# raymondclowe/EasyWakeWord

Hardware: NVIDIA B200
Metric: audio-sec/sec MFCC+cosine-match @4096 streams, 1/2/4/8 B200; % HBM peak (higher is better)
Workload: dtype f32

## Files before the change

easywakeword_b200/_lib.py:

```python
from __future__ import annotations

import ctypes as C
import os

import numpy as np

HERE = os.path.dirname(os.path.abspath(__file__))
LIB_PATH = os.path.join(HERE, "libewk.so")

EWK_OK, EWK_ERR_ARG, EWK_ERR_NO_TEMPLATE, EWK_ERR_CUDA, EWK_ERR_STATE, EWK_ERR_NOMEM = 0, -1, -2, -3, -4, -5
PCM_F32, PCM_I16 = 0, 1
IN_ULAW, IN_ALAW = 2, 3
HOST, DEVICE = 0, 1


class EwkError(RuntimeError):
    pass


class Config(C.Structure):
    _fields_ = [("n_streams", C.c_int32), ("ring_samples", C.c_int32), ("slack_samples", C.c_int32),
                ("pcm_format", C.c_int32), ("max_templates", C.c_int32), ("max_events", C.c_int32),
                ("preemphasis", C.c_float), ("n_mfcc", C.c_int32), ("reserved0", C.c_int32), ("reserved1", C.c_int32)]

# ... 267 lines not shown
        "ewk_push_g711": (C.c_int, [vp, i32, i32, vp, i64, i64, i32, i32]),
        "ewk_push_resampled": (C.c_int, [vp, i32, i32, vp, i32, i64, i64, i32, i32]),
        "ewk_push_resampled_each": (C.c_int, [vp, i32, i32, vp, i32, i64, i64, i32, i32, _p(i64)]),
        "ewk_push_streams": (C.c_int, [vp, _p(C.c_int32), i32, vp, i32, _p(i64), _p(i64), i64, i32, i32, _p(i64)]),
        "ewk_tick_ready": (C.c_int, [vp, i32, _p(C.c_int32), vp, vp, vp, vp]),
        "ewk_stream_input": (C.c_int, [vp, i32, _p(C.c_int32), _p(i64)]),
        "ewk_reset_streams": (C.c_int, [vp, _p(C.c_int32), i32]),
        "ewk_tick": (C.c_int, [vp, i32]),
        "ewk_set_overlap": (C.c_int, [vp, i32]),
        "ewk_join": (C.c_int, [vp]),
        "ewk_tick_trace": (C.c_int, [vp, i32, vp, vp, vp, vp]),
        "ewk_poll": (C.c_int, [vp, vp, i32, _p(C.c_int)]),
        "ewk_stream_status_get": (C.c_int, [vp, i32, _p(StreamStatus)]),
        "ewk_read_last": (C.c_int, [vp, i32, i64, f32p]),
        "ewk_read_segment": (C.c_int, [vp, i32, i64, i64, f32p]),
        "ewk_stream_results": (C.c_int, [vp, vp]),
        "ewk_dense_scores": (C.c_int, [vp, i64, i32, i32, i32, vp, i32]),
        "ewk_dense_scores_streams": (C.c_int, [vp, _p(C.c_int32), i32, _p(i64), _p(C.c_int32), i32, i32, vp, i64, i32]),
        "ewk_dense_ready": (C.c_int, [vp, _p(C.c_int32), i32, i32, i32, i32, _p(i64), _p(C.c_int32), vp, i64, i32]),
        "ewk_dense_detect": (C.c_int, [vp, _p(C.c_int32), i32, i32, i32, i32, i32, i32, vp, i32, _p(i64), _p(C.c_int32),
                                       vp, i64, i32]),
        "ewk_prepare_segments": (C.c_int, [vp, i32, _p(C.c_int32), _p(i64), _p(i64), _p(i64), f32p, i64, i32]),
        "ewk_results_device_ptr": (C.c_int, [vp, _p(vp)]),
        "ewk_set_results_buffer": (C.c_int, [vp, vp]),
        "ewk_set_results_peers": (C.c_int, [vp, _p(vp), i32, i64, i64, _p(vp), i32]),
        "ewk_publish_parity": (C.c_int, [vp]),
        "ewk_publish_seq": (C.c_int64, [vp]),
        "ewk_wait_published": (C.c_int, [vp, i32, i64, i32]),
        "ewk_published_seq": (C.c_int, [vp, i32, _p(C.c_uint64), i32]),
        "ewk_match_stream": (C.c_int, [vp, _p(vp)]),
        "ewk_host_alloc": (C.c_int, [_p(vp), i64]),
        "ewk_host_free": (C.c_int, [vp]),
        "ewk_launch_count": (C.c_int64, [vp]),
        "ewk_profile": (C.c_int, [vp, i32]),
        "ewk_profile_read": (C.c_int, [vp, _p(C.c_double), _p(C.c_int64)]),
    }
    for name, (res, args) in protos.items():
        fn = getattr(lib, name)
        fn.restype = res
        fn.argtypes = args
    lib._protos.update(protos)


_orig_load = load


def load():
    lib = _orig_load()
    if "ewk_push" not in lib._protos:
        _declare_stream_protos(lib)
    return lib


def default_stream_params(**over):
    lib = load()
    p = StreamParams()
    lib.ewk_default_stream_params(C.byref(p))
    for k, v in over.items():
        if not hasattr(p, k):
            raise TypeError(f"unknown stream parameter {k!r}")
        setattr(p, k, v)
    return p


class PinnedArray:

# ... 330 lines not shown
            signals = list(signals)
            if len(signals) != len(bases):
                raise ValueError("one signal row per destination")
            sig = (C.c_void_p * max(1, len(signals)))(*[C.c_void_p(int(b)) for b in signals])
        self._ck(self.lib.ewk_set_results_peers(self.h, arr, len(bases), int(stride_records), int(offset_records), sig, int(slot)))

    def publish_parity(self):
        return int(self.lib.ewk_publish_parity(self.h))

    def publish_seq(self):
        return int(self.lib.ewk_publish_seq(self.h))

    def wait_published(self, n_slots, seq, timeout_ms=2000):
        self._ck(self.lib.ewk_wait_published(self.h, int(n_slots), int(seq), int(timeout_ms)))

    def published_seq(self, parity, n_slots):
        out = np.zeros(n_slots, np.uint64)
        rc = self.lib.ewk_published_seq(self.h, int(parity), out.ctypes.data_as(_p(C.c_uint64)), int(n_slots))
        if rc < 0:
            self._ck(rc)
        return out, bool(rc)

    def match_stream(self):
        p = C.c_void_p()
        self._ck(self.lib.ewk_match_stream(self.h, C.byref(p)))
        return p.value or 0

    def set_cuda_stream(self, handle):
        self._ck(self.lib.ewk_set_cuda_stream(self.h, C.c_void_p(handle)))

    def launch_count(self):
        return int(self.lib.ewk_launch_count(self.h))

    def profile(self, enable=True):
        self._ck(self.lib.ewk_profile(self.h, 1 if enable else 0))

    def profile_read(self):
        ms = (C.c_double * 8)()
        n = (C.c_int64 * 8)()
        self._ck(self.lib.ewk_profile_read(self.h, ms, n))
        names = ["ring_push", "tick_gate", "segment_queue", "segment_batch", "dense_score", "segment_prepare", "publish",
                 "resample_push"]
        return {names[i]: {"ms": ms[i], "launches": int(n[i])} for i in range(len(names))}

    for f in (prepare_segments, dense_scores, dense_scores_streams, dense_ready, dense_detect, dense_last_plan, profile, profile_read, set_stream_params, push, push_g711, push_resampled,
              push_resampled_each, push_streams, tick_ready, reset_streams, stream_input, tick, poll, status, read_last, read_segment, results, results_device_ptr,
              set_results_buffer, set_results_peers, publish_parity, publish_seq, wait_published, published_seq, match_stream, set_cuda_stream, launch_count):
        setattr(Context, f.__name__, f)


_bank_methods()
```

easywakeword_b200/csrc/ewk_api.cu:

```cuda
#include <cuda_runtime.h>

#include <algorithm>
#include <cmath>
#include <climits>
#include <cstdarg>
#include <cstdio>
#include <cstdlib>
#include <cstring>
#include <string>
#include <type_traits>
#include <vector>

#include "../../include/ewk.h"
#include "ewk_ctx.hpp"

using namespace ewk;

static thread_local std::string g_create_error = "";

void ewk_ctx::fail(const char* fmt, ...) {
    char buf[1024];
    va_list ap;
    va_start(ap, fmt);
    vsnprintf(buf, sizeof(buf), fmt, ap);
// ... 516 lines not shown
    p->frame_size = 0;
    p->pre_speech_silence = 0.8;
    p->speech_duration_min = 0.3;
    p->speech_duration_max = 2.0;
    p->post_speech_silence = 0.4;
    p->timeout = 30.0;
    p->min_threshold = 0.005;
    p->template_first = 0;
    p->template_count = 1;
    p->live = 0;
    return EWK_OK;
}

int ewk_ctx::init_streams() {
    ewk_ctx* ctx = this;
    const int n = cfg.n_streams;
    if (n == 0) return EWK_OK;
    const size_t esz = cfg.pcm_format == EWK_PCM_I16 ? 2 : 4;
    bank.n_streams = n;
    bank.R = cfg.ring_samples;
    bank.P = ((cfg.ring_samples + cfg.slack_samples + 63) / 64) * 64;
    bank.fmt = cfg.pcm_format == EWK_PCM_I16 ? 1 : 0;
    chunk_cap = std::max(1, cfg.ring_samples / MIN_FRAME_SIZE);
    bank.chunk_cap = chunk_cap;
    bank.max_events = std::max(16, cfg.max_events);
    CK(cudaMalloc(&bank.ring, esz * (size_t)n * bank.P));
    CK(cudaMemsetAsync(bank.ring, 0, esz * (size_t)n * bank.P, stream));
    CK(cudaMalloc(&bank.st, sizeof(StreamState) * (size_t)n));
    CK(cudaMalloc(&bank.prm, sizeof(StreamParams) * (size_t)n));
    CK(cudaMalloc(&bank.chunk_ms, sizeof(double) * (size_t)n * 2 * chunk_cap));
    CK(cudaMalloc(&bank.events, sizeof(EventRec) * (size_t)bank.max_events));
    CK(cudaMalloc(&bank.ev_count, sizeof(int) * 8));
    CK(cudaMemsetAsync(bank.ev_count, 0, sizeof(int) * 8, stream));
    CK(cudaMalloc(&bank.bk_count, sizeof(int) * SEG_NB));
    CK(cudaMemsetAsync(bank.bk_count, 0, sizeof(int) * SEG_NB, stream));
    CK(cudaMalloc(&bank.bk_list, sizeof(int) * (size_t)SEG_NB * bank.max_events));
#ifdef EWK_K3_TRACE
    if (getenv("EWK_K3_TRACE")) {
        CK(cudaMalloc(&bank.k3_trace, sizeof(long long) * K3_TRACE_WORDS * (size_t)queue_grid()));
        CK(cudaMemsetAsync(bank.k3_trace, 0, sizeof(long long) * K3_TRACE_WORDS * (size_t)queue_grid(), stream));
    }
#endif

    bank.NB = bank.P / TICK;
    CK(cudaMalloc(&bank.block_ss, sizeof(double) * (size_t)n * std::max(1, bank.NB)));
    CK(cudaMalloc(&own_results, sizeof(StreamResult) * (size_t)n));
    bank.results = (StreamResult*)own_results;
    if (const char* e = getenv("EWK_K3")) k3_frames = atoi(e) == 2;
    if (!k3_frames) {
        if (use_lm) CK(cudaMalloc(&bank.lm_ws, sizeof(float) * (size_t)queue_grid() * SEG_SMEM_FRAMES * LM_ROW));
    } else {
        const size_t cap = std::min<size_t>((size_t)bank.max_events * SEG_SMEM_FRAMES, ((size_t)2 << 30) / (FROW * sizeof(float)));
        bank.frow_cap = (int)cap;
        CK(cudaMalloc(&bank.frow, sizeof(float) * FROW * cap));
        CK(cudaMalloc(&bank.frame_ev, sizeof(int) * cap));
        CK(cudaMalloc(&bank.ev_done, sizeof(int) * (size_t)bank.max_events));
    }
    std::vector<StreamState> st(n);
    std::memset(st.data(), 0, sizeof(StreamState) * n);
    for (auto& x : st) { x.thr = 0.01; x.last_ev = -1; }
    CK(cudaMemcpyAsync(bank.st, st.data(), sizeof(StreamState) * n, cudaMemcpyHostToDevice, stream));
    ewk_stream_params dp;
    ewk_default_stream_params(&dp);
    StreamParams sp;
    std::memcpy(&sp, &dp, sizeof(sp));
    h_prm.assign(n, sp);
    max_post = sp.post_speech_silence;
    CK(cudaMemcpyAsync(bank.prm, h_prm.data(), sizeof(StreamParams) * n, cudaMemcpyHostToDevice, stream));
    std::vector<StreamResult> rs(n);
    for (auto& r : rs) { r.score = std::nanf(""); r.flags = 0; }
    CK(cudaMemcpyAsync(bank.results, rs.data(), sizeof(StreamResult) * n, cudaMemcpyHostToDevice, stream));
    CK(cudaStreamSynchronize(stream));
    h_written.assign(n, 0);
    h_visible_lb.assign(n, 0);
    h_tick.assign(n, 0);
    h_dense_next.assign(n, 1);
    h_det_next.assign(n, 1);
    h_frame_size.assign(n, 0);
    h_rate.assign(n, 0);
    h_inputs.assign(n, 0);
    CK(cudaFuncSetAttribute(segment_queue_kernel<false>, cudaFuncAttributeMaxDynamicSharedMemorySize,
                            (int)seg_smem_bytes(SEG_SMEM_FRAMES)));
    CK(cudaFuncSetAttribute(segment_queue_kernel<true>, cudaFuncAttributeMaxDynamicSharedMemorySize,
                            (int)seg_smem_bytes(SEG_SMEM_FRAMES)));
    CK(cudaFuncSetAttribute(segment_frames_kernel<false>, cudaFuncAttributeMaxDynamicSharedMemorySize, (int)fq_smem_bytes()));
    CK(cudaFuncSetAttribute(segment_frames_kernel<true>, cudaFuncAttributeMaxDynamicSharedMemorySize, (int)fq_smem_bytes()));
    CK(cudaFuncSetAttribute(ring_push_bulk_kernel<short>, cudaFuncAttributeMaxDynamicSharedMemorySize, 112 * 1024));
    CK(cudaFuncSetAttribute(ring_push_bulk_kernel<float>, cudaFuncAttributeMaxDynamicSharedMemorySize, 112 * 1024));
    {
        const size_t big = sizeof(double) * 3 * (size_t)(std::min(chunk_cap, GATE_SMEM_CHUNKS) + 1) * GATE_WARPS;
        const size_t staged = sizeof(double) * 3 * (size_t)130 * GATE_WARPS + (size_t)2 * TICK * 4 * GATE_WARPS;
        CK(cudaFuncSetAttribute(tick_gate_kernel<false>, cudaFuncAttributeMaxDynamicSharedMemorySize, (int)std::max(big, staged)));
        CK(cudaFuncSetAttribute(tick_gate_kernel<true>, cudaFuncAttributeMaxDynamicSharedMemorySize, (int)std::max(big, staged)));
    }
    return EWK_OK;
}

void ewk_ctx::release_streams() {
#ifdef EWK_K3_TRACE
    if (bank.k3_trace) {
        cudaDeviceSynchronize();
        std::vector<long long> h((size_t)K3_TRACE_WORDS * queue_grid());
        cudaMemcpy(h.data(), bank.k3_trace, h.size() * sizeof(long long), cudaMemcpyDeviceToHost);
        if (FILE* f = fopen(getenv("EWK_K3_TRACE"), "wb")) { fwrite(h.data(), sizeof(long long), h.size(), f); fclose(f); }
        cudaFree(bank.k3_trace);
    }
#endif
    if (d_rs_tail) { cudaFree(d_rs_tail); d_rs_tail = nullptr; rs_tail_cap = 0; }
    for (void* p : {bank.ring, (void*)bank.st, (void*)bank.prm, (void*)bank.chunk_ms, (void*)bank.events,
                    (void*)bank.ev_count, (void*)bank.block_ss, (void*)bank.lm_ws, own_results, (void*)bank.frow,
                    (void*)bank.frame_ev, (void*)bank.ev_done, (void*)bank.bk_count, (void*)bank.bk_list})
        if (p) cudaFree(p);
    bank = BankView{};
    own_results = nullptr;
    b_trace.free(); b_read.free(); b_dense.free(); b_keep_rows.free(); b_keep_end.free(); b_g2.free(); b_det_state.free();
    for (auto& p : prof_pairs) { cudaEventDestroy(p.a); cudaEventDestroy(p.b); }
    for (auto e : prof_free) cudaEventDestroy(e);
    prof_pairs.clear(); prof_free.clear();
}

int ewk_ctx::gate_chunks() const {
    int m = 1;
    for (int s = 0; s < bank.n_streams; s++) {
        const int fs = h_frame_size[s] > 0 ? h_frame_size[s] : h_prm[s].frame_size;
        if (fs > 0) m = std::max(m, std::min(bank.chunk_cap, bank.R / fs));
    }
    return m;
}

int ewk_ctx::join_match() {
    ewk_ctx* ctx = this;
    if (!match_inflight) return EWK_OK;
    match_inflight = false;
    CK(cudaStreamWaitEvent(stream, ev_match, 0));
    return EWK_OK;
}

static int need_streams(ewk_ctx* ctx, const char* who, bool join = true) {
    if (ctx->bank.n_streams == 0) { ctx->fail("%s: context was created with n_streams = 0", who); return EWK_ERR_STATE; }
    if (join) return ctx->join_match();
    return EWK_OK;
}

extern "C" int ewk_set_overlap(ewk_ctx* ctx, int enable) {
    if (!ctx) return EWK_ERR_ARG;
    int rc = need_streams(ctx, "ewk_set_overlap");
    if (rc) return rc;
    CK(cudaSetDevice(ctx->device));
    if (enable && !ctx->match_stream) {
        CK(cudaStreamCreateWithFlags(&ctx->match_stream, cudaStreamNonBlocking));
        CK(cudaEventCreateWithFlags(&ctx->ev_gate, cudaEventDisableTiming));
        CK(cudaEventCreateWithFlags(&ctx->ev_match, cudaEventDisableTiming));
    }
    ctx->overlap = enable != 0;
    return EWK_OK;
}

extern "C" int ewk_join(ewk_ctx* ctx) {
    if (!ctx) return EWK_ERR_ARG;
    CK(cudaSetDevice(ctx->device));
    return ctx->join_match();
}

extern "C" int64_t ewk_launch_count(const ewk_ctx* ctx) { return ctx ? ctx->launches : 0; }

extern "C" int ewk_set_stream_params(ewk_ctx* ctx, int stream, const ewk_stream_params* p) {
    if (!ctx) return EWK_ERR_ARG;
    int rc = need_streams(ctx, "ewk_set_stream_params");
    if (rc) return rc;
    const int n = ctx->bank.n_streams;
    if (!p || stream < -1 || stream >= n) { ctx->fail("ewk_set_stream_params: bad stream %d", stream); return EWK_ERR_ARG; }
    if (!(p->pre_speech_silence > 0)) { ctx->fail("pre_speech_silence must be positive"); return EWK_ERR_ARG; }
    if (!(p->speech_duration_min > 0)) { ctx->fail("speech_duration_min must be positive"); return EWK_ERR_ARG; }
    if (!(p->speech_duration_max > 0)) { ctx->fail("speech_duration_max must be positive"); return EWK_ERR_ARG; }
    if (p->speech_duration_min > p->speech_duration_max) { ctx->fail("speech_duration_min must be <= speech_duration_max"); return EWK_ERR_ARG; }
    if (!(p->post_speech_silence > 0)) { ctx->fail("post_speech_silence must be positive"); return EWK_ERR_ARG; }
    if (p->frame_size != 0 && (p->frame_size < MIN_FRAME_SIZE || p->frame_size > ctx->bank.R)) {
        ctx->fail("frame_size must be 0 or in [%d, %d]", MIN_FRAME_SIZE, ctx->bank.R);
        return EWK_ERR_ARG;
    }
    if (p->template_first < 0 || p->template_count < 0 || p->template_first + p->template_count > ctx->cfg.max_templates) {
        ctx->fail("template range [%d, %d) outside [0, %d)", p->template_first, p->template_first + p->template_count, ctx->cfg.max_templates);
        return EWK_ERR_ARG;
    }
    CK(cudaSetDevice(ctx->device));
    StreamParams sp;
    std::memcpy(&sp, p, sizeof(sp));
    const int a = stream < 0 ? 0 : stream, b = stream < 0 ? n : stream + 1;
    for (int s = a; s < b; s++) ctx->h_prm[s] = sp;
    ctx->max_post = 0.0;
    for (int s = 0; s < n; s++) ctx->max_post = std::max(ctx->max_post, ctx->h_prm[s].post_speech_silence);
    CK(cudaMemcpyAsync(ctx->bank.prm + a, ctx->h_prm.data() + a, sizeof(StreamParams) * (size_t)(b - a),
                       cudaMemcpyHostToDevice, ctx->stream));
    CK(cudaStreamSynchronize(ctx->stream));
    return EWK_OK;
}

// ... 675 lines not shown
    const bool want = silent || state || thr || rms;
    const size_t cells = (size_t)B.n_streams * n_ticks;
    if (want) {
        CK(ctx->b_trace.ensure(cells * (2 + 16)));
        char* base = (char*)ctx->b_trace.p;
        tr.thr = (double*)base;
        tr.rms = (double*)(base + cells * 8);
        tr.silent = (unsigned char*)(base + cells * 16);
        tr.state = (unsigned char*)(base + cells * 17);
        if (paced) CK(cudaMemsetAsync(ctx->b_trace.p, 0xFF, cells * (2 + 16), ctx->stream));
    }
    int smem_chunks = ctx->gate_chunks();
    if (smem_chunks > GATE_SMEM_CHUNKS) {
        ctx->fail("ewk_tick: ring_samples / frame_size = %d chunks; the gate keeps them in shared memory and supports at most %d "
                  "(use a larger frame_size or a shorter ring)", smem_chunks, GATE_SMEM_CHUNKS);
        return EWK_ERR_ARG;
    }
    if (smem_chunks & 1) smem_chunks++;
    static const int stage_env = [] { const char* e = getenv("EWK_GATE_STAGE"); return e ? atoi(e) : 1; }();
    const int stage_bytes = (stage_env && smem_chunks <= 128 && !ctx->all_presummed) ? TICK * (B.fmt == 1 ? 2 : 4) : 0;
    if (B.n_pub > 0) {
        ctx->publish_seq++;
        B.pub_seq = (unsigned long long)ctx->publish_seq;
        B.pub_parity = (int)((ctx->publish_seq - 1) & 1);
    }
    if (B.n_pub > 0 && ctx->ev_pub_valid[B.pub_parity])
        CK(cudaStreamWaitEvent(ctx->stream, ctx->ev_pub[B.pub_parity], 0));
    cudaEvent_t pe = ctx->prof_begin(1);
    for (int done = 0; done < rounds_ticks; done += GATE_MAX_TICKS) {
        const int nt = std::min(GATE_MAX_TICKS, rounds_ticks - done);
        auto k2 = paced ? tick_gate_kernel<true> : tick_gate_kernel<false>;
        k2<<<(B.n_streams + GATE_WARPS - 1) / GATE_WARPS, GATE_THREADS,
             sizeof(double) * 3 * (size_t)smem_chunks * GATE_WARPS + (size_t)2 * stage_bytes * GATE_WARPS,
             ctx->stream>>>(B, nt, tr, n_ticks, done, smem_chunks, stage_bytes);
        ctx->launches++;
    }
    ctx->prof_end(pe, 1);
    CK(cudaGetLastError());
    const int grid = ctx->queue_grid();
    cudaStream_t ks = ctx->stream;
    const long long drop_reserve = (long long)std::ceil((ctx->max_post + 0.15) * 16000.0);
    if (ctx->overlap && (long long)B.R >= MAX_SEG + (long long)(rounds_ticks + 2) * TICK + drop_reserve && !want) {
        CK(cudaEventRecord(ctx->ev_gate, ctx->stream));
        CK(cudaStreamWaitEvent(ctx->match_stream, ctx->ev_gate, 0));
        ks = ctx->match_stream;
    }
    ctx->last_match_stream = ks;
    pe = ctx->prof_begin(2, ks);
    if (ctx->k3_frames) {
        auto k3f = ctx->cfg.preemphasis != 0.f ? segment_frames_kernel<true> : segment_frames_kernel<false>;
        k3f<<<grid, SEG_THREADS, fq_smem_bytes(), ks>>>(ctx->d_tables, B, ctx->d_tmpl, ctx->cfg.max_templates);
    } else {
        auto k3q = ctx->cfg.preemphasis != 0.f ? segment_queue_kernel<true> : segment_queue_kernel<false>;
        k3q<<<grid, SEG_THREADS, seg_smem_bytes(SEG_SMEM_FRAMES), ks>>>(ctx->d_tables, B, ctx->d_tmpl, ctx->cfg.max_templates);
    }
    ctx->prof_end(pe, 2, ks);
    CK(cudaGetLastError());
    if (ks != ctx->stream) {
        CK(cudaEventRecord(ctx->ev_match, ks));
        ctx->match_inflight = true;
    }
    ctx->launches += 1;
    if (B.n_pub > 0) {
        CK(cudaEventRecord(ctx->ev_k3, ks));
        CK(cudaStreamWaitEvent(ctx->pub_stream, ctx->ev_k3, 0));
        cudaEvent_t pp = ctx->prof_begin(6, ctx->pub_stream);
        publish_records_kernel<<<B.n_pub, 256, 0, ctx->pub_stream>>>(B);
// ... 800 lines not shown
```

easywakeword_b200/csrc/ewk_ctx.hpp:

```cpp
#pragma once
#include <cuda_runtime.h>

#include <map>
#include <string>
#include <vector>

#include "ewk_frame.cuh"
#include "ewk_segment.cuh"
#include "ewk_streams.cuh"
#include "ewk_dense.cuh"
#include "ewk_vad.cuh"
#include "ewk_resample.cuh"
#include "ewk_resample_push.cuh"
#include "ewk_tables.hpp"

#define EWK_MAX_TEMPLATES 64

namespace ewk {

struct DevBuf {
    void* p = nullptr;
    size_t cap = 0;
    cudaError_t ensure(size_t bytes) {
        if (bytes <= cap) return cudaSuccess;
        if (p) cudaFree(p);
        p = nullptr; cap = 0;
        size_t want = bytes + bytes / 4 + 256;
        cudaError_t e = cudaMalloc(&p, want);
        if (e == cudaSuccess) cap = want;
        return e;
    }
    void free() { if (p) cudaFree(p); p = nullptr; cap = 0; }
};

}

struct ewk_ctx {
    int device = 0;
    int sm_count = 0;
    bool use_lm = true;
    bool k3_frames = false;
    ewk_config cfg{};
    std::string err;
    cudaStream_t own_stream = nullptr, stream = nullptr, copy_stream = nullptr;
    cudaEvent_t ev_ready[2] = {nullptr, nullptr}, ev_free[2] = {nullptr, nullptr};
    bool ev_free_valid[2] = {false, false};
    cudaStream_t match_stream = nullptr;
    cudaEvent_t ev_gate = nullptr, ev_match = nullptr;
    bool overlap = false, match_inflight = false;
    long long publish_seq = 0;
    int* d_wait_flag = nullptr;
    cudaStream_t pub_stream = nullptr;
    cudaEvent_t ev_k3 = nullptr, ev_pub[2] = {nullptr, nullptr};
    bool ev_pub_valid[2] = {false, false};
    void* d_pub_snap = nullptr;
    cudaStream_t last_match_stream = nullptr;
    int join_match();
    int stage_idx = 0;
    struct Pending {
        bool valid = false; int slot = 0, stream0 = 0, n_streams = 0; long long n = 0;
        int rs_rate = 0, rs_fmt = 0; long long rs_n_in = 0, rs_c = 0;
        int rows_slot = -1; long long n_items = 0; std::vector<ewk::RowDesc> rows;
    } pending;
    int land(int stream0, int n_streams, const void* d_src, long long d_stride, long long n, int stage_slot);
    int land_resampled(int stream0, int n_streams, const void* d_src, long long d_stride, int in_fmt, long long n_in,
                       int sr_in, long long c, const ewk::RowDesc* rows, int rows_slot, long long n_items, int stage_slot);
    int land_list(const std::vector<ewk::RowDesc>& rows, int rows_slot, long long n_items, const void* d_src, int in_fmt,
                  int stage_slot);
    int upload_rows(const std::vector<ewk::RowDesc>& rows, cudaStream_t on, int* slot);
    ewk::RowDesc* h_pos[2] = {nullptr, nullptr};
    ewk::DevBuf b_pos[2];
    cudaEvent_t ev_pos[2] = {nullptr, nullptr};
    bool ev_pos_valid[2] = {false, false};
    int pos_idx = 0;
// ... 71 lines not shown
```

easywakeword_b200/csrc/ewk_streams.cuh:

```cuda
#pragma once
#include "ewk_frame.cuh"
#include "ewk_segment.cuh"

#ifndef EWK_MAX_TEMPLATES
#define EWK_MAX_TEMPLATES 64
#endif

namespace ewk {

constexpr int GATE_THREADS = 128;
constexpr int TICK = 1600;
constexpr int MAX_SEG = 48000;

enum : int { ST_WAITING = 0, ST_IN_SILENCE = 1, ST_IN_SOUND = 2, ST_AFTER_SOUND = 3 };
enum : int { EV_PENDING = 0, EV_TIMEOUT = 1, EV_SCORED = 2 };

struct StreamParams {
    float similarity_threshold;
    int frame_size;
    double pre_speech_silence, speech_duration_min, speech_duration_max, post_speech_silence;
    double timeout;
    double min_threshold;
    int template_first, template_count;
    int live;
// ... 25 lines not shown
    long long seg_start;
    int seg_len;
    int tmpl;
    float score;
    int matched;
};

struct StreamResult {
    float score;
    unsigned flags;
};

constexpr int MAX_PUB = 16;
constexpr int SEG_NB = 24;
constexpr int FROW = 24;

struct BankView {
    void* ring;
    StreamState* st;
    StreamParams* prm;
    double* chunk_ms;
    EventRec* events;
    int* ev_count;
    int* frame_ev;
    int* ev_done;
    float* frow;
    int frow_cap;
    StreamResult* results;
    double* block_ss;
    float* lm_ws;
    int* bk_count;
    int* bk_list;
    long long* k3_trace;
    int n_streams, R, P, fmt, chunk_cap, max_events, NB;
    StreamResult* pub[MAX_PUB];
    int n_pub, pub_parity;
    long long pub_stride, pub_off;
    unsigned long long* pub_sig[MAX_PUB];
    unsigned long long pub_seq;
    int pub_slot;
    int pad_pub;
    StreamResult* pub_snap;
};

__global__ void __launch_bounds__(256)
publish_records_kernel(BankView B) {
    const int p = blockIdx.x;
    const unsigned long long* src = reinterpret_cast<const unsigned long long*>(B.pub_snap + (size_t)B.pub_parity * B.n_streams);
    unsigned long long* dst = reinterpret_cast<unsigned long long*>(B.pub[p] + (size_t)B.pub_parity * (size_t)B.pub_stride + (size_t)B.pub_off);
    for (int i0 = threadIdx.x; i0 < B.n_streams; i0 += 8 * blockDim.x) {
        unsigned long long v[8];
#pragma unroll
        for (int u = 0; u < 8; u++) { const int i = i0 + u * blockDim.x; v[u] = i < B.n_streams ? __ldcg(src + i) : 0ull; }
#pragma unroll
        for (int u = 0; u < 8; u++) {
            const int i = i0 + u * blockDim.x;
            if (i < B.n_streams) asm volatile("st.weak.global.b64 [%0], %1;" :: "l"(dst + i), "l"(v[u]) : "memory");
        }
    }
    __threadfence_system();
    __syncthreads();
    if (threadIdx.x == 0 && B.pub_sig[p]) {
        unsigned long long* sg = B.pub_sig[p] + (size_t)B.pub_parity * MAX_PUB + B.pub_slot;
        asm volatile("st.release.sys.global.u64 [%0], %1;" :: "l"(sg), "l"(B.pub_seq) : "memory");
    }
}
// ... 342 lines not shown
#pragma unroll
            for (int r = 0; r < 4; r++) {
                const int i = 32 * r + lane;
                if (i >= pos_new && i < pos_old) S[i + 1] = __longlong_as_double(v[r]);
            }
        }
        __syncwarp();
        if (lane == 0) S[pos_new] = newv;
        __syncwarp();
        return;
    }
    int lo = 0, ln = 0;
    for (int i0 = 0; i0 < n; i0 += 32) {
        const int i = i0 + lane;
        const long long v = i < n ? __double_as_longlong(S[i]) : 0x7fffffffffffffffLL;
        lo += __popc(__ballot_sync(FULL, v < bo));
        ln += __popc(__ballot_sync(FULL, v < bn));
    }
    const int pos_old = lo;
    const int pos_new = ln - (bo < bn ? 1 : 0);
    for (int i = lane; i < n; i += 32) {
        double v;
        if (i == pos_new) v = newv;
        else {
            const int r = i > pos_new ? i - 1 : i;
            v = S[r >= pos_old ? r + 1 : r];
        }
        T[i] = v;
    }
    __syncwarp();
    double* t = S; S = T; T = t;
}

__device__ __forceinline__ double percentile25_rms_sorted(const double* S, int n) {
    const double vi = (double)n * 0.25 - 0.25;
    const int k_lo = (int)floor(vi);
    const int k_hi = min(k_lo + 1, n - 1);
    const double a = sqrt(S[k_lo]), b = sqrt(S[k_hi]);
    const double t = vi - (double)k_lo;
    const double diff = __dsub_rn(b, a);
    double r = __dadd_rn(a, __dmul_rn(diff, t));
    if (t >= 0.5) r = __dsub_rn(b, __dmul_rn(diff, __dsub_rn(1.0, t)));
    return r;
}

__device__ __forceinline__ unsigned smem_u32(const void* p) { return (unsigned)__cvta_generic_to_shared(p); }
__device__ __forceinline__ void mbar_init(unsigned long long* bar, unsigned count) {
    asm volatile("mbarrier.init.shared::cta.b64 [%0], %1;" ::"r"(smem_u32(bar)), "r"(count) : "memory");
}
__device__ __forceinline__ void mbar_expect_tx(unsigned long long* bar, unsigned bytes) {
    asm volatile("mbarrier.arrive.expect_tx.release.cta.shared::cta.b64 _, [%0], %1;" ::"r"(smem_u32(bar)), "r"(bytes) : "memory");
}
__device__ __forceinline__ void bulk_g2s(void* dst, const void* src, unsigned bytes, unsigned long long* bar) {
    asm volatile("cp.async.bulk.shared::cta.global.mbarrier::complete_tx::bytes [%0], [%1], %2, [%3];"
                 ::"r"(smem_u32(dst)), "l"(src), "r"(bytes), "r"(smem_u32(bar)) : "memory");
}
__device__ __forceinline__ void mbar_wait(unsigned long long* bar, unsigned parity) {
    unsigned done = 0;
    while (!done) {
        asm volatile("{\n\t.reg .pred p;\n\tmbarrier.try_wait.parity.shared::cta.b64 p, [%1], %2;\n\tselp.b32 %0, 1, 0, p;\n\t}"
                     : "=r"(done) : "r"(smem_u32(bar)), "r"(parity) : "memory");
    }
}

__device__ __forceinline__ double warp_sumsq_smem(const void* buf, int fmt, int lane) {
    double acc;
    if (fmt == 1) {
        const int4* v = reinterpret_cast<const int4*>(buf);
        long long iacc = 0;
#pragma unroll
        for (int u = 0; u < 7; u++) {
            const int k = lane + 32 * u;
            if (k < TICK / 8) iacc += sq8(v[k]);
        }
        acc = (double)iacc;
    } else {
// ... 49 lines not shown
    int j = 0, b = 0, st = 0, p0 = 0, bi = 0;
    unsigned phase = 0;
    for (long long k = 0; k < my_items; k++) {
        const int s = stream0 + gw + j * GW;
        if (b == 0) {
            const long long w_cur = w_next;
            p0 = (int)(w_cur % B.P);
            bi = (int)((w_cur / TICK) % B.NB);
            if (j + 1 < my_streams) w_next = B.st[s + GW].written;
        }
        mbar_wait(full + st, phase);
        const double acc = warp_sumsq_smem(buf + (size_t)st * BYTES, sizeof(T) == 2 ? 1 : 0, lane);
        asm volatile("fence.proxy.async.shared::cta;" ::: "memory");
        __syncwarp();
        if (lane == 0) {
            bulk_s2g((T*)B.ring + (size_t)s * B.P + p0, buf + (size_t)st * BYTES, BYTES);
            asm volatile("cp.async.bulk.commit_group;" ::: "memory");
            B.block_ss[(size_t)s * B.NB + bi] = acc;
            if (k >= 1) {
                asm volatile("cp.async.bulk.wait_group.read 1;" ::: "memory");
                issue();
            }
        }
        __syncwarp();
        if (++st == stages) { st = 0; phase ^= 1u; }
        p0 += TICK; if (p0 >= B.P) p0 -= B.P;
        if (++bi == B.NB) bi = 0;
        if (++b == nb) { b = 0; j++; }
    }
    if (lane == 0) asm volatile("cp.async.bulk.wait_group 0;" ::: "memory");
}

struct GatePlan {
    long long V[GATE_MAX_TICKS];
    double pv[GATE_MAX_TICKS][GATE_MAXP + 1];
    short pc[GATE_MAX_TICKS][GATE_MAXP];
    unsigned char np[GATE_MAX_TICKS];
    unsigned char alias[GATE_MAX_TICKS];
    unsigned char full[GATE_MAX_TICKS];
    double rms[GATE_MAX_TICKS];
};

__device__ __forceinline__ unsigned gate_state_step(const BankView& B, int s, StreamState& st, const StreamParams& prm,
                                                    long long k, long long V, bool full, int silent) {
    unsigned evflag = 0;
    const double now = __dmul_rn((double)k, 0.1);
    if (full && !st.started) {
        st.started = 1;
        st.state = silent ? ST_IN_SILENCE : ST_WAITING;
        st.start_time = now;
        if (silent) st.silence_start = now;
        return 0;
    }
    if (!st.started) return 0;
    const double prev = __dmul_rn((double)(k - 1), 0.1);
    if (prm.timeout > 0.0 && __dsub_rn(prev, st.start_time) > prm.timeout) {
        const int idx = atomicAdd(B.ev_count, 1);
        if (idx < B.max_events) {
            EventRec e{};
            e.stream = s; e.kind = EV_TIMEOUT; e.tick = k - 1; e.score = __int_as_float(0x7fc00000);
            B.events[idx] = e;
        } else { atomicAdd(B.ev_count + 1, 1); atomicSub(B.ev_count, 1); }
        st.n_timeouts++;
        st.state = st.last_silent ? ST_IN_SILENCE : ST_WAITING;
        st.start_time = prev;
        if (st.last_silent) st.silence_start = prev;
// ... 36 lines not shown
                            e.stream = s; e.kind = EV_PENDING; e.tick = k;
                            e.seg_start = V - n_back; e.seg_len = (int)len;
                            e.tmpl = f0;
                            e.score = __int_as_float(0x7fc00000); e.matched = 0;
                            B.events[idx] = e;
                            if (B.frame_ev) {
                                B.ev_done[idx] = 0;
                                for (int t = 0; t < nf; t++) B.frame_ev[f0 + t] = idx;
                            }
                            {
                                const int b = min(SEG_NB - 1, (nf + SEG_WARPS - 1) / SEG_WARPS);
                                const int q = atomicAdd(B.bk_count + b, 1);
                                if (q < B.max_events) B.bk_list[(size_t)b * B.max_events + q] = idx;
                            }
                            st.n_events++;
                            st.last_ev = idx;
                            evflag = 16u;
                        } else {
                            atomicAdd(B.ev_count + 1, 1); atomicSub(B.ev_count, 1);
                            if (B.frame_ev && f0 >= 0)
                                for (int t = 0; t < nf && f0 + t < B.frow_cap; t++) B.frame_ev[f0 + t] = -1;
                        }
                    }
                    st.state = ST_WAITING;
                }
            } else st.state = ST_WAITING;
            break;
    }
    return evflag;
}

template <bool PACED>
__global__ void __launch_bounds__(GATE_THREADS, 7)
tick_gate_kernel(BankView B, int n_ticks, TraceView tr, int trace_stride, int trace_off, int smem_chunks, int stage_bytes) {
    extern __shared__ __align__(16) double sm_d[];
    __shared__ GatePlan plans[GATE_WARPS];
    __shared__ __align__(8) unsigned long long mbar[GATE_WARPS][2];
    char* stage = reinterpret_cast<char*>(sm_d + (size_t)GATE_WARPS * 3 * smem_chunks);
    __shared__ StreamState st_s[GATE_WARPS];
    __shared__ StreamParams prm_s[GATE_WARPS];
    const int tid = threadIdx.x, lane = tid & 31, warp = tid >> 5;
    const int s = blockIdx.x * GATE_WARPS + warp;
    if (s >= B.n_streams) return;
    double* ms = sm_d + (size_t)warp * 3 * smem_chunks;
    double* SA = ms + smem_chunks;
    double* SB = SA + smem_chunks;
    GatePlan& plan = plans[warp];

    StreamState& st = st_s[warp];
    const StreamParams& prm = prm_s[warp];
    double* g_ms = B.chunk_ms + (size_t)s * 2 * B.chunk_cap;
    double* g_sorted = g_ms + B.chunk_cap;
    {
        static_assert(sizeof(StreamState) % 8 == 0 && sizeof(StreamParams) % 8 == 0, "8-byte words");
        const unsigned long long* gs = reinterpret_cast<const unsigned long long*>(B.st + s);
        const unsigned long long* gp = reinterpret_cast<const unsigned long long*>(B.prm + s);
        unsigned long long* ds = reinterpret_cast<unsigned long long*>(&st_s[warp]);
        unsigned long long* dp = reinterpret_cast<unsigned long long*>(&prm_s[warp]);
        if (lane < (int)(sizeof(StreamState) / 8)) ds[lane] = gs[lane];
        if (lane < (int)(sizeof(StreamParams) / 8)) dp[lane] = gp[lane];
        const int spec = min(smem_chunks, B.chunk_cap);
        for (int i = lane; i < spec; i += 32) { ms[i] = g_ms[i]; SA[i] = g_sorted[i]; }
    }
    __syncwarp();
    if (PACED) n_ticks = (int)max(0LL, min((long long)n_ticks, st.written / TICK - st.tick));
    const int fs = st.frame_size;
    const long long tick0 = st.tick, visible0 = st.visible, written0 = st.written;
// ... 23 lines not shown
            if (upd) {
                const long long dv = V - Vp;
                if (!valid_before || dv >= B.R) np = 255;
                else {
                    const int q0 = (int)(Vp % B.R);
                    const long long e = q0 + dv;
                    const int e1 = (int)min(e, (long long)B.R);
                    const int c1 = q0 / fs;
                    const int n1 = (e1 - 1) / fs - c1 + 1;
                    const int n2 = e > B.R ? (int)((e - B.R - 1) / fs) + 1 : 0;
                    for (int i = 0; i < n1 + n2; i++) {
                        const int c = i < n1 ? c1 + i : i - n1;
                        if (c >= n_chunks) continue;
                        if (np == GATE_MAXP) { np = 255; break; }
                        plan.pc[j][np++] = (short)c;
                    }
                    if (np == 1 && fs == TICK && dv == TICK && (q0 % TICK) == 0 && B.R >= TICK) alias = 1;
                }
            }
            plan.V[j] = V;
            plan.full[j] = full;
            plan.np[j] = (unsigned char)np;
            plan.alias[j] = (unsigned char)alias;
        }
    }
    __syncwarp();

    const int nrec = min(TICK, B.R);
    unsigned evflag = 0;
    int valid = valid0;
    long long key_lo = -1, key_hi = -1;

    bool rms_ahead = false;
    auto replay_tick = [&](int j) {
        const long long k = tick0 + j + 1;
        const long long V = plan.V[j];
        const bool full = plan.full[j];
        const int np = plan.np[j];
        if (np == 255) {
            for (int c = 0; c < n_chunks; c++) {
                const double v = warp_chunk_ms(B, s, V, fs, c, lane);
                if (lane == 0) ms[c] = v;
            }
            __syncwarp();
            warp_sort_build(ms, SA, n_chunks, lane);
            valid = 1;
        } else {
            for (int i = 0; i < np; i++) {
                const int c = plan.pc[j][i];
                const double nv = plan.pv[j][i];
                const double ov = ms[c];
                __syncwarp();
                warp_sorted_replace(SA, SB, n_chunks, ov, nv, lane);
                if (lane == 0) ms[c] = nv;
                __syncwarp();
            }
        }
        if (lane == 0) {
            if (np != 0) {
                const int k_lo = (int)floor((double)n_chunks * 0.25 - 0.25), k_hi = min(k_lo + 1, n_chunks - 1);
                const long long b_lo = __double_as_longlong(SA[k_lo]), b_hi = __double_as_longlong(SA[k_hi]);
                if (b_lo != key_lo || b_hi != key_hi) {
                    key_lo = b_lo; key_hi = b_hi;
                    const double p25 = percentile25_rms_sorted(SA, n_chunks);
                    const double nt = __dmul_rn(p25, 1.5);
                    st.thr = nt > prm.min_threshold ? nt : prm.min_threshold;
                }
            }
            int silent = 1;
            double rms = 0.0;
            if (fs > 0) {
                if (rms_ahead) rms = plan.rms[j];
                else {
                    double ss;
                    if (plan.alias[j]) ss = plan.pv[j][0] * (double)fs;
                    else { ss = plan.pv[j][GATE_MAXP]; if (B.fmt == 1) ss *= (1.0 / 1073741824.0); }
                    rms = sqrt(ss / (double)nrec);
                }
                silent = rms < st.thr;
            }
            st.last_rms = rms;
            evflag |= gate_state_step(B, s, st, prm, k, V, full, silent);
            st.last_silent = silent;
            if (tr.silent) {
                const size_t o = (size_t)s * trace_stride + trace_off + j;
                tr.silent[o] = (unsigned char)silent;
                tr.state[o] = (unsigned char)(st.started ? st.state : 255);
                tr.thr[o] = st.thr;
                tr.rms[o] = rms;
            }
            st.tick = k; st.visible = V;
        }
    };

    const size_t esz = B.fmt == 1 ? 2 : 4;
    const bool mine_ok = lane >= n_ticks || (plan.alias[lane] && plan.np[lane] == 1);
    const bool all_alias = (B.P % TICK) == 0 && __all_sync(FULL, mine_ok);
    const bool presummed = all_alias && B.NB > 0 && n_ticks > 0 && plan.V[0] - TICK >= st.ss_from;
    if (presummed) {
        if (lane < n_ticks) {
            double ss = B.block_ss[(size_t)s * B.NB + (size_t)(((plan.V[lane] - TICK) / TICK) % B.NB)];
            if (B.fmt == 1) ss *= (1.0 / 1073741824.0);
            plan.pv[lane][0] = ss / (double)fs;
        }
        __syncwarp();
    }
    const bool pipelined = !presummed && stage_bytes > 0 && all_alias && (!PACED || n_ticks > 0);
    unsigned long long* bar = mbar[warp];
    char* buf = stage + (size_t)warp * 2 * stage_bytes;
    const char* ring_s = (const char*)B.ring + (size_t)s * B.P * esz;
    int pos0 = 0;
    auto issue = [&](int j) {
        int pos = pos0 + j * TICK;
        while (pos >= B.P) pos -= B.P;
        mbar_expect_tx(bar + (j & 1), (unsigned)(TICK * esz));
        bulk_g2s(buf + (size_t)(j & 1) * stage_bytes, ring_s + (size_t)pos * esz, (unsigned)(TICK * esz), bar + (j & 1));
    };
    if (pipelined) {
        pos0 = (int)((plan.V[0] - TICK) % B.P);
        if (lane == 0) {
            mbar_init(bar, 1); mbar_init(bar + 1, 1);
            asm volatile("fence.mbarrier_init.release.cluster;" ::: "memory");
            issue(0);
            if (n_ticks > 1) issue(1);
        }
        __syncwarp();
    } else if (!presummed) {
        for (int j = 0; j < n_ticks; j++) {
            const long long V = plan.V[j];
            const int np = plan.np[j] == 255 ? 0 : plan.np[j];
            for (int i = 0; i < np; i++) {
                const double v = warp_chunk_ms(B, s, V, fs, plan.pc[j][i], lane);
                if (lane == 0) plan.pv[j][i] = v;
            }
            if (fs > 0 && !plan.alias[j]) {
                const long long a0 = V - nrec;
                const double ss = warp_sumsq(ring_s, B.P, B.fmt, a0 < 0 ? 0 : a0, (int)(a0 < 0 ? V : nrec), lane);
                if (lane == 0) plan.pv[j][GATE_MAXP] = ss;
            }
        }
        __syncwarp();
    }
    if (!pipelined) {
        if (lane < n_ticks && fs > 0) {
            double ss;
            if (plan.alias[lane]) ss = plan.pv[lane][0] * (double)fs;
            else { ss = plan.pv[lane][GATE_MAXP]; if (B.fmt == 1) ss *= (1.0 / 1073741824.0); }
            plan.rms[lane] = sqrt(ss / (double)nrec);
        }
        rms_ahead = true;
        __syncwarp();
    }
    for (int j = 0; j < n_ticks; j++) {
        if (pipelined) {
            mbar_wait(bar + (j & 1), (unsigned)((j >> 1) & 1));
            double ss = warp_sumsq_smem(buf + (size_t)(j & 1) * stage_bytes, B.fmt, lane);
            __syncwarp();
            if (lane == 0) {
                if (j + 2 < n_ticks) {
                    asm volatile("fence.proxy.async.shared::cta;" ::: "memory");
                    issue(j + 2);
                }
                if (B.fmt == 1) ss *= (1.0 / 1073741824.0);
                plan.pv[j][0] = ss / (double)fs;
            }
            __syncwarp();
        }
        replay_tick(j);
    }
    __syncwarp();

    if (use_chunks && valid)
        for (int i = lane; i < n_chunks; i += 32) { g_ms[i] = ms[i]; g_sorted[i] = SA[i]; }
    if (lane == 0) {
        st.chunks_valid = valid;
        B.st[s] = st;
        StreamResult r = B.results[s];
        r.flags = (r.flags & 1u) | (st.last_silent ? 2u : 0u) | ((unsigned)st.state << 2) | evflag |
                  ((unsigned)st.n_events << 8);
        store_result(B.results + s, r);
        if (B.n_pub) store_result(B.pub_snap + (size_t)B.pub_parity * B.n_streams + s, r);
    }
}

struct PrepDesc { int stream; int len; long long start; long long out_off; };

__global__ void __launch_bounds__(256)
segment_prepare_kernel(BankView B, const PrepDesc* __restrict__ d, float* __restrict__ out) {
    __shared__ double red[8];
    __shared__ double bc[2];
    const PrepDesc pd = d[blockIdx.x];
    const int tid = threadIdx.x, lane = tid & 31, warp = tid >> 5;
    const short* q = B.fmt == 1 ? (const short*)B.ring + (size_t)pd.stream * B.P : nullptr;
    const float* f = B.fmt == 0 ? (const float*)B.ring + (size_t)pd.stream * B.P : nullptr;
    const int p0 = (int)(pd.start % B.P);
    auto at = [&](int i) -> double {
        int p = p0 + i;
        if (p >= B.P) p -= B.P;
        return q ? (double)q[p] * (1.0 / 32768.0) : (double)f[p];
    };
    double s = 0.0;
    for (int i = tid; i < pd.len; i += 256) s += at(i);
#pragma unroll
    for (int o = 16; o; o >>= 1) s += __shfl_xor_sync(FULL, s, o);
    if (lane == 0) red[warp] = s;
    __syncthreads();
    if (tid == 0) { double t = 0.0; for (int w = 0; w < 8; w++) t += red[w]; bc[0] = t / (double)pd.len; }
// ... 398 lines not shown
```

include/ewk.h:

```cpp
#ifndef EWK_H
#define EWK_H

#include <stdint.h>

#ifdef __cplusplus
extern "C" {
#endif

#define EWK_ABI_VERSION 2

typedef struct ewk_ctx ewk_ctx;

typedef enum ewk_status {
    EWK_OK = 0,
    EWK_ERR_ARG = -1,
    EWK_ERR_NO_TEMPLATE = -2,
    EWK_ERR_CUDA = -3,
    EWK_ERR_STATE = -4,
    EWK_ERR_NOMEM = -5
} ewk_status;

typedef enum ewk_pcm_format { EWK_PCM_F32 = 0, EWK_PCM_I16 = 1 } ewk_pcm_format;
typedef enum ewk_mem { EWK_HOST = 0, EWK_DEVICE = 1 } ewk_mem;

// ... 120 lines not shown
int ewk_push_resampled(ewk_ctx* ctx, int stream0, int n_streams, const void* in, int in_format, int64_t n_in, int64_t stride,
                       int where, int sr_in);
int ewk_push_resampled_each(ewk_ctx* ctx, int stream0, int n_streams, const void* in, int in_format, int64_t n_in,
                            int64_t stride, int where, int sr_in, int64_t* landed);
int ewk_push_streams(ewk_ctx* ctx, const int32_t* streams, int n, const void* in, int in_format,
                     const int64_t* offsets, const int64_t* lens, int64_t in_len, int where, int sr_in, int64_t* landed);
int ewk_tick_ready(ewk_ctx* ctx, int max_ticks, int32_t* taken, uint8_t* silent, uint8_t* state, double* thr, double* rms);
int ewk_stream_input(ewk_ctx* ctx, int stream, int32_t* sr_in, int64_t* n_in);
int ewk_reset_streams(ewk_ctx* ctx, const int32_t* streams, int n);
int ewk_dense_scores(ewk_ctx* ctx, int64_t hop0, int n_hops, int template_first, int template_count,
                     float* out, int where);
int ewk_dense_scores_streams(ewk_ctx* ctx, const int32_t* streams, int n, const int64_t* hop0, const int32_t* n_hops,
                             int template_first, int template_count, float* out, int64_t out_cap, int where);
int ewk_dense_ready(ewk_ctx* ctx, const int32_t* streams, int n, int max_hops, int template_first, int template_count,
                    int64_t* hop0_out, int32_t* n_hops_out, float* out, int64_t out_cap, int where);
int ewk_dense_detect(ewk_ctx* ctx, const int32_t* streams, int n, int max_hops, int template_first, int template_count,
                     int hold_hops, int refractory_hops, ewk_detection* det, int det_cap,
                     int64_t* hop0_out, int32_t* n_hops_out, float* out, int64_t out_cap, int where);
int ewk_dense_plan(const int64_t* template_lens, int n, int32_t out[4]);
int ewk_dense_last_plan(const ewk_ctx* ctx, int32_t out[4]);
int ewk_stream_results(ewk_ctx* ctx, ewk_stream_result* out);
int ewk_results_device_ptr(ewk_ctx* ctx, void** out);
int ewk_set_results_buffer(ewk_ctx* ctx, void* device_ptr);
int ewk_set_results_peers(ewk_ctx* ctx, void* const* bases, int n_bases, int64_t stride_records, int64_t offset_records,
                          void* const* signals, int slot);
int ewk_publish_parity(const ewk_ctx* ctx);
int64_t ewk_publish_seq(const ewk_ctx* ctx);
int ewk_wait_published(ewk_ctx* ctx, int n_slots, int64_t seq, int timeout_ms);
int ewk_published_seq(ewk_ctx* ctx, int parity, uint64_t* out, int n_slots);
int ewk_match_stream(ewk_ctx* ctx, void** out);
int ewk_host_alloc(void** out, int64_t bytes);
int ewk_host_free(void* p);
int64_t ewk_launch_count(const ewk_ctx* ctx);
enum { EWK_PROF_CLASSES = 8 };
int ewk_profile(ewk_ctx* ctx, int enable);
int ewk_profile_read(ewk_ctx* ctx, double* ms, int64_t* launches);

#ifdef __cplusplus
}
#endif
#endif
```

Baseline: 25.64 million.

## Parallelize tick-gate percentile replay across warp lanes with bitonic merge

Adds a warp-parallel fast path to the tick gate kernel. When each tick updates at most one distinct chunk, it runs a 64-element warp bitonic sort over the candidate window and rank counting, so the 25th-percentile thresholds for all ticks are computed at once instead of replaying ticks serially. It also writes the merged sorted array back in parallel. A serial fallback selected by environment variable, a per-stream fast flag, and a query API are added; the cost is more complexity and shared memory in GatePlan, which may reduce occupancy.

```diff
diff --git a/easywakeword_b200/_lib.py b/easywakeword_b200/_lib.py
--- a/easywakeword_b200/_lib.py
+++ b/easywakeword_b200/_lib.py
@@ -323,6 +323,7 @@
         "ewk_host_alloc": (C.c_int, [_p(vp), i64]),
         "ewk_host_free": (C.c_int, [vp]),
         "ewk_launch_count": (C.c_int64, [vp]),
+        "ewk_gate_fast_streams": (C.c_int, [vp, _p(C.c_int64)]),
         "ewk_profile": (C.c_int, [vp, i32]),
         "ewk_profile_read": (C.c_int, [vp, _p(C.c_double), _p(C.c_int64)]),
     }
@@ -719,6 +720,11 @@
     def launch_count(self):
         return int(self.lib.ewk_launch_count(self.h))
 
+    def gate_fast_streams(self):
+        out = C.c_int64()
+        self._ck(self.lib.ewk_gate_fast_streams(self.h, C.byref(out)))
+        return out.value
+
     def profile(self, enable=True):
         self._ck(self.lib.ewk_profile(self.h, 1 if enable else 0))
 
@@ -732,7 +738,8 @@
 
     for f in (prepare_segments, dense_scores, dense_scores_streams, dense_ready, dense_detect, dense_last_plan, profile, profile_read, set_stream_params, push, push_g711, push_resampled,
               push_resampled_each, push_streams, tick_ready, reset_streams, stream_input, tick, poll, status, read_last, read_segment, results, results_device_ptr,
-              set_results_buffer, set_results_peers, publish_parity, publish_seq, wait_published, published_seq, match_stream, set_cuda_stream, launch_count):
+              set_results_buffer, set_results_peers, publish_parity, publish_seq, wait_published, published_seq, match_stream, set_cuda_stream, launch_count,
+              gate_fast_streams):
         setattr(Context, f.__name__, f)
 
 
diff --git a/easywakeword_b200/csrc/ewk_api.cu b/easywakeword_b200/csrc/ewk_api.cu
--- a/easywakeword_b200/csrc/ewk_api.cu
+++ b/easywakeword_b200/csrc/ewk_api.cu
@@ -572,6 +572,8 @@
     CK(cudaMalloc(&bank.events, sizeof(EventRec) * (size_t)bank.max_events));
     CK(cudaMalloc(&bank.ev_count, sizeof(int) * 8));
     CK(cudaMemsetAsync(bank.ev_count, 0, sizeof(int) * 8, stream));
+    CK(cudaMalloc(&bank.gate_fast, (size_t)n));
+    CK(cudaMemsetAsync(bank.gate_fast, 0, (size_t)n, stream));
     CK(cudaMalloc(&bank.bk_count, sizeof(int) * SEG_NB));
     CK(cudaMemsetAsync(bank.bk_count, 0, sizeof(int) * SEG_NB, stream));
     CK(cudaMalloc(&bank.bk_list, sizeof(int) * (size_t)SEG_NB * bank.max_events));
@@ -587,6 +589,7 @@
     CK(cudaMalloc(&own_results, sizeof(StreamResult) * (size_t)n));
     bank.results = (StreamResult*)own_results;
     if (const char* e = getenv("EWK_K3")) k3_frames = atoi(e) == 2;
+    if (const char* e = getenv("EWK_GATE_REPLAY")) gate_serial = std::strcmp(e, "serial") == 0;
     if (!k3_frames) {
         if (use_lm) CK(cudaMalloc(&bank.lm_ws, sizeof(float) * (size_t)queue_grid() * SEG_SMEM_FRAMES * LM_ROW));
     } else {
@@ -649,7 +652,7 @@
     if (d_rs_tail) { cudaFree(d_rs_tail); d_rs_tail = nullptr; rs_tail_cap = 0; }
     for (void* p : {bank.ring, (void*)bank.st, (void*)bank.prm, (void*)bank.chunk_ms, (void*)bank.events,
                     (void*)bank.ev_count, (void*)bank.block_ss, (void*)bank.lm_ws, own_results, (void*)bank.frow,
-                    (void*)bank.frame_ev, (void*)bank.ev_done, (void*)bank.bk_count, (void*)bank.bk_list})
+                    (void*)bank.frame_ev, (void*)bank.ev_done, (void*)bank.bk_count, (void*)bank.bk_list, (void*)bank.gate_fast})
         if (p) cudaFree(p);
     bank = BankView{};
     own_results = nullptr;
@@ -703,6 +706,18 @@
 }
 
 extern "C" int64_t ewk_launch_count(const ewk_ctx* ctx) { return ctx ? ctx->launches : 0; }
+
+extern "C" int ewk_gate_fast_streams(ewk_ctx* ctx, int64_t* out) {
+    if (!ctx || !out) return EWK_ERR_ARG;
+    *out = 0;
+    if (ctx->bank.n_streams == 0) return EWK_OK;
+    CK(cudaSetDevice(ctx->device));
+    std::vector<unsigned char> h((size_t)ctx->bank.n_streams);
+    CK(cudaMemcpyAsync(h.data(), ctx->bank.gate_fast, h.size(), cudaMemcpyDeviceToHost, ctx->stream));
+    CK(cudaStreamSynchronize(ctx->stream));
+    for (unsigned char f : h) *out += f;
+    return EWK_OK;
+}
 
 extern "C" int ewk_set_stream_params(ewk_ctx* ctx, int stream, const ewk_stream_params* p) {
     if (!ctx) return EWK_ERR_ARG;
@@ -1444,7 +1459,7 @@
         auto k2 = paced ? tick_gate_kernel<true> : tick_gate_kernel<false>;
         k2<<<(B.n_streams + GATE_WARPS - 1) / GATE_WARPS, GATE_THREADS,
              sizeof(double) * 3 * (size_t)smem_chunks * GATE_WARPS + (size_t)2 * stage_bytes * GATE_WARPS,
-             ctx->stream>>>(B, nt, tr, n_ticks, done, smem_chunks, stage_bytes);
+             ctx->stream>>>(B, nt, tr, n_ticks, done, smem_chunks, stage_bytes, ctx->gate_serial ? 1 : 0);
         ctx->launches++;
     }
     ctx->prof_end(pe, 1);
diff --git a/easywakeword_b200/csrc/ewk_ctx.hpp b/easywakeword_b200/csrc/ewk_ctx.hpp
--- a/easywakeword_b200/csrc/ewk_ctx.hpp
+++ b/easywakeword_b200/csrc/ewk_ctx.hpp
@@ -40,6 +40,7 @@
     int sm_count = 0;
     bool use_lm = true;
     bool k3_frames = false;
+    bool gate_serial = false;
     ewk_config cfg{};
     std::string err;
     cudaStream_t own_stream = nullptr, stream = nullptr, copy_stream = nullptr;
diff --git a/easywakeword_b200/csrc/ewk_streams.cuh b/easywakeword_b200/csrc/ewk_streams.cuh
--- a/easywakeword_b200/csrc/ewk_streams.cuh
+++ b/easywakeword_b200/csrc/ewk_streams.cuh
@@ -81,6 +81,7 @@
     int* bk_count;
     int* bk_list;
     long long* k3_trace;
+    unsigned char* gate_fast;
     int n_streams, R, P, fmt, chunk_cap, max_events, NB;
     StreamResult* pub[MAX_PUB];
     int n_pub, pub_parity;
@@ -489,16 +490,41 @@
     double* t = S; S = T; T = t;
 }
 
-__device__ __forceinline__ double percentile25_rms_sorted(const double* S, int n) {
+__device__ __forceinline__ double percentile25_rms(double lo_ms, double hi_ms, int n) {
     const double vi = (double)n * 0.25 - 0.25;
     const int k_lo = (int)floor(vi);
-    const int k_hi = min(k_lo + 1, n - 1);
-    const double a = sqrt(S[k_lo]), b = sqrt(S[k_hi]);
+    const double a = sqrt(lo_ms), b = sqrt(hi_ms);
     const double t = vi - (double)k_lo;
     const double diff = __dsub_rn(b, a);
     double r = __dadd_rn(a, __dmul_rn(diff, t));
     if (t >= 0.5) r = __dsub_rn(b, __dmul_rn(diff, __dsub_rn(1.0, t)));
     return r;
+}
+__device__ __forceinline__ double percentile25_rms_sorted(const double* S, int n) {
+    const int k_lo = (int)floor((double)n * 0.25 - 0.25);
+    return percentile25_rms(S[k_lo], S[min(k_lo + 1, n - 1)], n);
+}
+
+__device__ __forceinline__ void warp_bitonic64(long long& a, long long& b, int lane) {
+#pragma unroll
+    for (int k = 2; k <= 64; k <<= 1) {
+#pragma unroll
+        for (int j = k >> 1; j > 0; j >>= 1) {
+            if (j == 32) {
+                const long long lo = a < b ? a : b, hi = a < b ? b : a;
+                a = lo; b = hi;
+                continue;
+            }
+#pragma unroll
+            for (int r = 0; r < 2; r++) {
+                long long& v = r ? b : a;
+                const int i = 32 * r + lane;
+                const long long p = __shfl_xor_sync(FULL, v, j);
+                const bool take_min = ((i & j) == 0) == ((i & k) == 0);
+                v = take_min ? (p < v ? p : v) : (p < v ? v : p);
+            }
+        }
+    }
 }
 
 __device__ __forceinline__ unsigned smem_u32(const void* p) { return (unsigned)__cvta_generic_to_shared(p); }
@@ -614,6 +640,8 @@
 }
 
 struct GatePlan {
+    longlong2 onv[GATE_MAX_TICKS];
+    double thr[GATE_MAX_TICKS];
     long long V[GATE_MAX_TICKS];
     double pv[GATE_MAX_TICKS][GATE_MAXP + 1];
     short pc[GATE_MAX_TICKS][GATE_MAXP];
@@ -716,7 +744,8 @@
 
 template <bool PACED>
 __global__ void __launch_bounds__(GATE_THREADS, 7)
-tick_gate_kernel(BankView B, int n_ticks, TraceView tr, int trace_stride, int trace_off, int smem_chunks, int stage_bytes) {
+tick_gate_kernel(BankView B, int n_ticks, TraceView tr, int trace_stride, int trace_off, int smem_chunks, int stage_bytes,
+                 int serial_replay) {
     extern __shared__ __align__(16) double sm_d[];
     __shared__ GatePlan plans[GATE_WARPS];
     __shared__ __align__(8) unsigned long long mbar[GATE_WARPS][2];
@@ -806,10 +835,37 @@
     long long key_lo = -1, key_hi = -1;
 
     bool rms_ahead = false;
-    auto replay_tick = [&](int j) {
+    auto finish_tick = [&](int j) {
         const long long k = tick0 + j + 1;
         const long long V = plan.V[j];
         const bool full = plan.full[j];
+        int silent = 1;
+        double rms = 0.0;
+        if (fs > 0) {
+            if (rms_ahead) rms = plan.rms[j];
+            else {
+                double ss;
+                if (plan.alias[j]) ss = plan.pv[j][0] * (double)fs;
+                else { ss = plan.pv[j][GATE_MAXP]; if (B.fmt == 1) ss *= (1.0 / 1073741824.0); }
+                rms = sqrt(ss / (double)nrec);
+            }
+            silent = rms < st.thr;
+        }
+        st.last_rms = rms;
+        evflag |= gate_state_step(B, s, st, prm, k, V, full, silent);
+        st.last_silent = silent;
+        if (tr.silent) {
+            const size_t o = (size_t)s * trace_stride + trace_off + j;
+            tr.silent[o] = (unsigned char)silent;
+            tr.state[o] = (unsigned char)(st.started ? st.state : 255);
+            tr.thr[o] = st.thr;
+            tr.rms[o] = rms;
+        }
+        st.tick = k; st.visible = V;
+    };
+
+    auto replay_tick = [&](int j) {
+        const long long V = plan.V[j];
         const int np = plan.np[j];
         if (np == 255) {
             for (int c = 0; c < n_chunks; c++) {
@@ -841,29 +897,7 @@
                     st.thr = nt > prm.min_threshold ? nt : prm.min_threshold;
                 }
             }
-            int silent = 1;
-            double rms = 0.0;
-            if (fs > 0) {
-                if (rms_ahead) rms = plan.rms[j];
-                else {
-                    double ss;
-                    if (plan.alias[j]) ss = plan.pv[j][0] * (double)fs;
-                    else { ss = plan.pv[j][GATE_MAXP]; if (B.fmt == 1) ss *= (1.0 / 1073741824.0); }
-                    rms = sqrt(ss / (double)nrec);
-                }
-                silent = rms < st.thr;
-            }
-            st.last_rms = rms;
-            evflag |= gate_state_step(B, s, st, prm, k, V, full, silent);
-            st.last_silent = silent;
-            if (tr.silent) {
-                const size_t o = (size_t)s * trace_stride + trace_off + j;
-                tr.silent[o] = (unsigned char)silent;
-                tr.state[o] = (unsigned char)(st.started ? st.state : 255);
-                tr.thr[o] = st.thr;
-                tr.rms[o] = rms;
-            }
-            st.tick = k; st.visible = V;
+            finish_tick(j);
         }
     };
 
@@ -925,7 +959,86 @@
         rms_ahead = true;
         __syncwarp();
     }
-    for (int j = 0; j < n_ticks; j++) {
+    bool fast = false;
+    if (!serial_replay && !pipelined && valid0 && use_chunks && n_ticks > 0) {
+        const int np = lane < n_ticks ? plan.np[lane] : 0;
+        const int key = np == 1 ? (int)plan.pc[lane][0] : -1 - lane;
+        const unsigned same = __match_any_sync(FULL, key);
+        fast = __all_sync(FULL, np <= 1 && same == (1u << lane));
+    }
+    if (fast) {
+        constexpr long long NONE = 0x7fffffffffffffffLL;
+        const bool upd = lane < n_ticks && plan.np[lane] == 1;
+        const int c_mine = upd ? plan.pc[lane][0] : 0;
+        const long long ov_mine = upd ? __double_as_longlong(ms[c_mine]) : NONE;
+        const long long nv_mine = upd ? __double_as_longlong(plan.pv[lane][0]) : NONE;
+        if (lane < GATE_MAX_TICKS) plan.onv[lane] = make_longlong2(ov_mine, nv_mine);
+        const unsigned updmask = __ballot_sync(FULL, upd);
+        const int m = __popc(updmask);
+        auto count_le = [&](long long x) {
+            int lo = 0, hi = n_chunks;
+            while (lo < hi) {
+                const int mid = (lo + hi) >> 1;
+                if (__double_as_longlong(SA[mid]) <= x) lo = mid + 1; else hi = mid;
+            }
+            return lo;
+        };
+        const int k_lo = (int)floor((double)n_chunks * 0.25 - 0.25), k_hi = min(k_lo + 1, n_chunks - 1);
+        const int w0 = max(0, k_lo - m), nw = min(n_chunks - 1, k_hi + m) - w0 + 1;
+        auto candidate = [&](int i) {
+            const long long nv = __shfl_sync(FULL, nv_mine, max(0, min(31, i - nw)));
+            return i < nw ? __double_as_longlong(SA[w0 + i]) : i < nw + n_ticks ? nv : NONE;
+        };
+        long long x0 = candidate(lane), x1 = candidate(32 + lane);
+        warp_bitonic64(x0, x1, lane);
+        __syncwarp();
+        int n0 = count_le(x0), n1 = count_le(x1);
+        long long lo_mine = 0, hi_mine = 0;
+        for (int j = 0; j < n_ticks; j++) {
+            const longlong2 on = plan.onv[j];
+            n0 += (on.y <= x0) - (on.x <= x0);
+            n1 += (on.y <= x1) - (on.x <= x1);
+            const unsigned a_lo = __ballot_sync(FULL, n0 > k_lo), b_lo = __ballot_sync(FULL, n1 > k_lo);
+            const unsigned a_hi = __ballot_sync(FULL, n0 > k_hi), b_hi = __ballot_sync(FULL, n1 > k_hi);
+            const int p_lo = a_lo ? __ffs(a_lo) - 1 : 31 + __ffs(b_lo);
+            const int p_hi = a_hi ? __ffs(a_hi) - 1 : 31 + __ffs(b_hi);
+            const long long v_lo = __shfl_sync(FULL, p_lo < 32 ? x0 : x1, p_lo & 31);
+            const long long v_hi = __shfl_sync(FULL, p_hi < 32 ? x0 : x1, p_hi & 31);
+            if (lane == j) { lo_mine = v_lo; hi_mine = v_hi; }
+        }
+        if (lane < n_ticks) {
+            double thr = st.thr;
+            if (updmask & ((2u << lane) - 1u)) {
+                const double p25 = percentile25_rms(__longlong_as_double(lo_mine), __longlong_as_double(hi_mine), n_chunks);
+                const double nt = __dmul_rn(p25, 1.5);
+                thr = nt > prm.min_threshold ? nt : prm.min_threshold;
+            }
+            plan.thr[lane] = thr;
+        }
+        __syncwarp();
+        if (lane == 0)
+            for (int j = 0; j < n_ticks; j++) { st.thr = plan.thr[j]; finish_tick(j); }
+        if (upd) g_ms[c_mine] = __longlong_as_double(nv_mine);
+        for (int p = lane; p < n_chunks; p += 32) {
+            const long long x = __double_as_longlong(SA[p]);
+            int o_lt = 0, o_eq = 0, n_lt = 0;
+            for (int j = 0; j < n_ticks; j++) {
+                const longlong2 on = plan.onv[j];
+                o_lt += on.x < x; o_eq += on.x == x; n_lt += on.y < x;
+            }
+            if (o_eq == 0 || (p + o_eq < n_chunks && __double_as_longlong(SA[p + o_eq]) == x))
+                g_sorted[p - o_lt + n_lt] = __longlong_as_double(x);
+        }
+        if (upd) {
+            int pos = count_le(nv_mine);
+            for (int j = 0; j < n_ticks; j++) {
+                const longlong2 on = plan.onv[j];
+                pos += (on.y < nv_mine || (on.y == nv_mine && j < lane)) - (on.x <= nv_mine);
+            }
+            g_sorted[pos] = __longlong_as_double(nv_mine);
+        }
+    }
+    for (int j = 0; j < n_ticks && !fast; j++) {
         if (pipelined) {
             mbar_wait(bar + (j & 1), (unsigned)((j >> 1) & 1));
             double ss = warp_sumsq_smem(buf + (size_t)(j & 1) * stage_bytes, B.fmt, lane);
@@ -944,9 +1057,10 @@
     }
     __syncwarp();
 
-    if (use_chunks && valid)
+    if (use_chunks && valid && !fast)
         for (int i = lane; i < n_chunks; i += 32) { g_ms[i] = ms[i]; g_sorted[i] = SA[i]; }
     if (lane == 0) {
+        if (B.gate_fast) B.gate_fast[s] = fast;
         st.chunks_valid = valid;
         B.st[s] = st;
         StreamResult r = B.results[s];
diff --git a/include/ewk.h b/include/ewk.h
--- a/include/ewk.h
+++ b/include/ewk.h
@@ -176,6 +176,7 @@
 int ewk_host_alloc(void** out, int64_t bytes);
 int ewk_host_free(void* p);
 int64_t ewk_launch_count(const ewk_ctx* ctx);
+int ewk_gate_fast_streams(ewk_ctx* ctx, int64_t* out);
 enum { EWK_PROF_CLASSES = 8 };
 int ewk_profile(ewk_ctx* ctx, int enable);
 int ewk_profile_read(ewk_ctx* ctx, double* ms, int64_t* launches);
```

Measured after the change: 24.70 million (median of 6 runs). 0.964x the previous value.
